# JunweiLiang/Multiverse

Measured on AMD Instinct MI355X. Metric: trajectories/sec (8-obs/12-pred, multi-scale 18x32+9x16 grid, greedy forward), higher is better.
Workload: dtype f16x3 (fp32 operands as two pre-scaled fp16 planes, fp32 accumulate and state; winograd F(3,3) over image rows on pre-transformed operands, 1.67 fp16 MFMAs issued per fp32 product over the gate kernels; error vs fp64 within 2x of the fp32-MFMA path's -- asserted under checkpoint-like dynamic range (; 1 GPU; BASELINE configs[1]: multi-scale 18x32+9x16 (scene 36x64x11), batch 64/GPU, fp32 forward-only, beam 1, obs 8 / pred 12; gate convolution on the fp16 matrix pipe (f16x3 split, fp32-class error); batch_per_gpu=64, global_batch=64, obs_len=8, pred_len=12, parallelism=batch-sharded x1, no data-path collective

## Files before the change

multiverse_amd/csrc/decode_tail.h:

```cpp
#pragma once
#include <hip/hip_runtime.h>
#include <stdint.h>

#include "convlstm_mfma.h"
#include "kernels_misc.h"
#include "plane_layout.h"

namespace mv {

constexpr int kTailMax = 4;

__global__ void pack_h2g_kernel(const float* __restrict__ w, float* __restrict__ wq, int C,
                                int P) {
  const int idx = blockIdx.x * blockDim.x + threadIdx.x;
  if (idx >= C * 32) return;
  const int j = idx & 3, l = (idx >> 2) & 63, kk = idx >> 8;
  const int c = kk * 8 + (l >> 5) * 4 + j, col = l & 31;
  float v = 0.f;
  if (col < 9 * P) {
    const int tap = col / P, p = col - tap * P;
    v = w[((size_t)tap * C + c) * P + p];
  }
  wq[idx] = v;
}

struct H2gQProblem {
  const float* h;
  const float* wq;
  float* q;
  int32_t cells, P;
};
struct H2gQGroup {
  H2gQProblem p[kTailMax];
  int32_t block_end[kTailMax];
  int32_t n;
};

template <int NK>
__device__ __forceinline__ void h2g_q_body(const H2gQProblem& a, int block, int C, float* wl) {
  const int lane = threadIdx.x & 63, wave = threadIdx.x >> 6;
  {
    const f32x4* wg = reinterpret_cast<const f32x4*>(a.wq);
    f32x4* wd = reinterpret_cast<f32x4*>(wl);
    for (int i = threadIdx.x; i < C * 8; i += 256) wd[i] = wg[i];
  }
  __syncthreads();
  const int m_wave = block * 128 + wave * 32;
  if (m_wave >= a.cells) return;
  const int m = m_wave + (lane & 31);
  const float* src = a.h + (size_t)(m < a.cells ? m : 0) * C + (lane >> 5) * 4;
  const f32x4* wsrc = reinterpret_cast<const f32x4*>(wl) + lane;
  f32x16 acc;
#pragma unroll
  for (int i = 0; i < 16; ++i) acc[i] = 0.f;
  for (int c0 = 0; c0 < C; c0 += NK * 8) {
    f32x4 av[NK];
#pragma unroll
    for (int kk = 0; kk < NK; ++kk) av[kk] = *reinterpret_cast<const f32x4*>(src + c0 + kk * 8);
    __builtin_amdgcn_sched_barrier(0);
#pragma unroll
    for (int kk = 0; kk < NK; ++kk) {
      const f32x4 bv = wsrc[((c0 >> 3) + kk) * 64];
#pragma unroll
      for (int j = 0; j < 4; ++j)
        acc = __builtin_amdgcn_mfma_f32_32x32x2f32(av[kk][j], bv[j], acc, 0, 0, 0);
    }
  }
  const int col = lane & 31, QS = 9 * a.P;
  if (col < QS) {
#pragma unroll
    for (int reg = 0; reg < 16; ++reg) {
      const int row = (reg & 3) + 8 * (reg >> 2) + 4 * (lane >> 5);
      const int mm = m_wave + row;
      if (mm < a.cells) a.q[(size_t)mm * QS + col] = acc[reg];
    }
  }
}

template <int NK>
__global__ __launch_bounds__(256)
void h2g_q_kernel(const H2gQGroup g, int C) {
  extern __shared__ __attribute__((aligned(16))) float h2g_wlds[];
  int block = blockIdx.x;
  int pi = 0;
#pragma unroll
  for (int i = 0; i < kTailMax - 1; ++i)
    if (i + 1 < g.n && (int)blockIdx.x >= g.block_end[i]) pi = i + 1;
  if (pi > 0) block -= g.block_end[pi - 1];
  switch (pi) {
    case 0: h2g_q_body<NK>(g.p[0], block, C, h2g_wlds); break;
    case 1: h2g_q_body<NK>(g.p[1], block, C, h2g_wlds); break;
    case 2: h2g_q_body<NK>(g.p[2], block, C, h2g_wlds); break;
    default: h2g_q_body<NK>(g.p[3], block, C, h2g_wlds); break;
  }
}

static inline void launch_h2g_q(const H2gQProblem* probs, int n, int C, hipStream_t stream) {
  H2gQGroup g{};
  g.n = n;
  unsigned total = 0;
  for (int i = 0; i < n; ++i) {
    g.p[i] = probs[i];
    total += (unsigned)((probs[i].cells + 127) / 128);
    g.block_end[i] = (int32_t)total;
  }
  for (int i = n; i < kTailMax; ++i) g.block_end[i] = (int32_t)total;
  const size_t lds = (size_t)C * 128;
  if (C % 256 == 0)
    hipLaunchKernelGGL(h2g_q_kernel<32>, dim3(total), dim3(256), lds, stream, g, C);
  else
    hipLaunchKernelGGL(h2g_q_kernel<16>, dim3(total), dim3(256), lds, stream, g, C);
}

__device__ __forceinline__ void emb_store8(float* __restrict__ x, _Float16* p16, size_t pst,
                                           size_t m, int c8, int E, const float (&v)[8]) {
  f32x4 lo = {v[0], v[1], v[2], v[3]}, hi = {v[4], v[5], v[6], v[7]};
  f32x4* dst = reinterpret_cast<f32x4*>(x + m * E + c8 * 8);
  dst[0] = lo; dst[1] = hi;
  if (p16) {
    typedef _Float16 h8 __attribute__((ext_vector_type(8)));
    h8 a, b;
    const size_t o = plane_index((long long)m, c8 * 8, E);
    if (pst == 0) {
#pragma unroll
      for (int j = 0; j < 8; ++j) a[j] = bf16_half_bits(v[j]);
      *reinterpret_cast<h8*>(p16 + o) = a;
      return;
    }
#pragma unroll
    for (int j = 0; j < 8; ++j) {
      const float s = v[j] * 256.0f;
      const _Float16 h0 = (_Float16)s;
      a[j] = h0;
      b[j] = (_Float16)(s - (float)h0);
    }
    *reinterpret_cast<h8*>(p16 + o) = a;
    *reinterpret_cast<h8*>(p16 + pst + o) = b;
  }
}

__global__ __launch_bounds__(256)
void grid_emb_onehot8_kernel(const int32_t* __restrict__ ids, int ids_stride, int ids_div,
                             const float* __restrict__ w, const float* __restrict__ b,
                             float* __restrict__ out, int M, int H, int W, int E,
                             _Float16* p16, size_t p16_stride, int act = 0) {
  const int ng = E >> 3;
  const size_t item = (size_t)blockIdx.x * blockDim.x + threadIdx.x;
  const int K = H * W;
  if (item >= (size_t)M * K * ng) return;
  const int c8 = (int)(item % ng);
  const size_t mc = item / ng;
  const int m = (int)(mc / K), cell = (int)(mc - (size_t)m * K);
  const int yy = cell / W, xx = cell - yy * W;
  const int id = ids[(size_t)(m / ids_div) * ids_stride];
  const int py = id / W, px = id - py * W;
  const int dy = yy - py, dx = xx - px;
  const bool hot = dy >= -1 && dy <= 1 && dx >= -1 && dx <= 1;
  const float* wp = w + (hot ? (1 - dy) * 3 + (1 - dx) : 4) * E + c8 * 8;
  float v[8];
#pragma unroll
  for (int j = 0; j < 8; ++j) {
    const float acc = hot ? wp[j] : 0.f;
    v[j] = act_apply(act, acc + b[c8 * 8 + j]);
  }
  emb_store8(out, p16, p16_stride, mc, c8, E, v);
}

struct TailProblem {
  const float* q;
  float* out;
  int64_t out_row_stride;
  int32_t* ids_out;
  const float* emb_w;
  const float* emb_b;
  float* x_out;
  _Float16* x16;
  int64_t x16_stride;
  int32_t rows, H, W, P, E;
  int32_t onehot;
  int32_t act;
};
struct TailGroup {
  TailProblem p[kTailMax];
  int32_t block_end[kTailMax];
  int32_t n;
};

__device__ __forceinline__ void decode_tail_body(const TailProblem& a, int row, float* sm) {
  const int tid = threadIdx.x, lane = tid & 63, wave = tid >> 6;
  const int H = a.H, W = a.W, K = H * W, P = a.P, E = a.E, QS = 9 * P;
  float* vals = sm;
  float* wl = sm + 2 * 1024;
  float* red = wl + 9 * 2 * E;
  int* redi = reinterpret_cast<int*>(red + 16);
  const float* qrow = a.q + (size_t)row * K * QS;
  if (a.emb_w && !a.onehot)
    for (int i = tid; i < 9 * P * E; i += blockDim.x) wl[i] = a.emb_w[i];
  float best = -INFINITY;
  int bi = 0x7fffffff;
  for (int idx = tid; idx < K * P; idx += blockDim.x) {
    const int cell = idx / P, p = idx - cell * P;
    const int y = cell / W, x = cell - y * W;
    float acc = 0.f;
#pragma unroll
    for (int t = 0; t < 9; ++t) {
      const int yy = y + t / 3 - 1, xx = x + t % 3 - 1;
      if (yy >= 0 && yy < H && xx >= 0 && xx < W)
        acc += qrow[(size_t)(yy * W + xx) * QS + t * P + p];
    }
    vals[idx] = acc;
    a.out[(size_t)row * a.out_row_stride + idx] = acc;
    if (acc > best || (acc == best && idx < bi)) { best = acc; bi = idx; }
  }
  if (!a.emb_w && !a.ids_out) return;
  int hot = 0;
  if (a.onehot) {
#pragma unroll
    for (int off = 32; off > 0; off >>= 1) {
      const float ov = __shfl_xor(best, off, 64);
      const int oi = __shfl_xor(bi, off, 64);
      if (ov > best || (ov == best && oi < bi)) { best = ov; bi = oi; }
    }
    if (lane == 0) { red[wave] = best; redi[wave] = bi; }
    __syncthreads();
    best = red[0]; bi = redi[0];
    for (int wv = 1; wv < (int)(blockDim.x >> 6); ++wv) {
      const float ov = red[wv];
      const int oi = redi[wv];
      if (ov > best || (ov == best && oi < bi)) { best = ov; bi = oi; }
    }
    hot = bi;
    if (a.ids_out && tid == 0) a.ids_out[row] = hot;
  } else {
    __syncthreads();
  }
  if (!a.emb_w) return;
  const int ng = E >> 3;
  const int py = hot / W, px = hot - py * W;
  for (int item = tid; item < K * ng; item += blockDim.x) {
    const int cell = item / ng, c8 = item - cell * ng;
    const int y = cell / W, x = cell - y * W;
    float v[8];
    if (a.onehot) {
      const int dy = y - py, dx = x - px;
      const bool in = dy >= -1 && dy <= 1 && dx >= -1 && dx <= 1;
      const float* wp = a.emb_w + (in ? (1 - dy) * 3 + (1 - dx) : 4) * E + c8 * 8;
#pragma unroll
      for (int j = 0; j < 8; ++j) v[j] = act_apply(a.act, (in ? wp[j] : 0.f) + a.emb_b[c8 * 8 + j]);
    } else {
      float acc[8];
#pragma unroll
      for (int j = 0; j < 8; ++j) acc[j] = 0.f;
      for (int t = 0; t < 9; ++t) {
        const int yy = y + t / 3 - 1, xx = x + t % 3 - 1;
        if (yy < 0 || yy >= H || xx < 0 || xx >= W) continue;
        const float* ip = vals + (yy * W + xx) * P;
        for (int p = 0; p < P; ++p) {
          const float iv = ip[p];
          const float* wp = wl + (t * P + p) * E + c8 * 8;
#pragma unroll
          for (int j = 0; j < 8; ++j) acc[j] = fmaf(iv, wp[j], acc[j]);
        }
      }
#pragma unroll
      for (int j = 0; j < 8; ++j) v[j] = act_apply(a.act, acc[j] + a.emb_b[c8 * 8 + j]);
    }
    emb_store8(a.x_out, a.x16, (size_t)a.x16_stride, (size_t)row * K + cell, c8, E, v);
  }
}

static inline size_t tail_lds_bytes(int E) {
  return ((size_t)2 * 1024 + (size_t)9 * 2 * E + 32) * sizeof(float);
}
constexpr int kTailThreads = 1024;

__global__ __launch_bounds__(kTailThreads)
void decode_tail_kernel(const TailGroup g) {
  extern __shared__ __attribute__((aligned(16))) float tail_sm[];
  int block = blockIdx.x;
  int pi = 0;
#pragma unroll
  for (int i = 0; i < kTailMax - 1; ++i)
    if (i + 1 < g.n && (int)blockIdx.x >= g.block_end[i]) pi = i + 1;
  if (pi > 0) block -= g.block_end[pi - 1];
  switch (pi) {
    case 0: decode_tail_body(g.p[0], block, tail_sm); break;
    case 1: decode_tail_body(g.p[1], block, tail_sm); break;
    case 2: decode_tail_body(g.p[2], block, tail_sm); break;
    default: decode_tail_body(g.p[3], block, tail_sm); break;
  }
}

static inline void launch_decode_tail(const TailProblem* probs, int n, hipStream_t stream) {
  TailGroup g{};
  g.n = n;
  unsigned total = 0;
  for (int i = 0; i < n; ++i) {
    g.p[i] = probs[i];
    total += (unsigned)probs[i].rows;
    g.block_end[i] = (int32_t)total;
  }
  for (int i = n; i < kTailMax; ++i) g.block_end[i] = (int32_t)total;
  int emax = 32;
  for (int i = 0; i < n; ++i) emax = probs[i].E > emax ? probs[i].E : emax;
  hipLaunchKernelGGL(decode_tail_kernel, dim3(total), dim3(kTailThreads), tail_lds_bytes(emax),
                     stream, g);
}

}
```

multiverse_amd/csrc/engine_forward.h:

```cpp
#pragma once

namespace {


using mv::ConvLstmArgs;

void set_sparse_x(mv_engine* e, ScaleState& S, ConvLstmArgs& a, bool decoder,
                  const int32_t* hot, int hot_stride, int hot_div) {
  a.sx_bias = decoder ? S.sx_dec_bias.p : nullptr;
  a.sx_corr = decoder ? S.sx_dec_corr.p : S.sx_enc_corr.p;
  a.sx_hot = hot; a.sx_hot_stride = hot_stride; a.sx_hot_div = hot_div;
  a.sx_cellyx = S.sx_cellyx.p;
  a.sx_rad = decoder ? 2 : 1;
  a.sx_by_class = decoder ? 1 : 0;
}

ConvLstmArgs conv_problem(mv_engine* e, const ConvCell& cc, const float* x,
                          const float* h, const float* c, const int32_t* src_row_h,
                          const int32_t* src_row_c, float* h_out, float* c_out,
                          int rows, int H, int W, bool zero_state,
                          size_t x_row_stride = 0, bool want_h16 = true) {
  ConvLstmArgs a{};
  const size_t xrs = x_row_stride ? x_row_stride : (size_t)H * W * cc.Cx;
  MV_REQUIRE((size_t)rows * H * W * e->cfg.hidden_size < ((size_t)1 << 31) &&
// ... 243 lines not shown
    launch(e, "wino3_transform", 0, tr3_bytes, [&] {
      mv::launch_wino3_transforms(tr3.data(), (int)tr3.size(), e->issue);
    });
  launch(e, "convlstm_step", g.flops, g.bytes, [&] {
    launch_gate_group(pl, g.p16.data(), packs, w_hwio, v3x, v3h, n, e->issue);
  }, g.dense, pl.mfma_factor);
}

void run_conv_group_f16x3(mv_engine* e, const std::vector<ConvLstmArgs>& probs) {
  const GatePrep g = prepare_gate_group(e, probs);
  const GatePrep* gp = &g;
  issue_gate_group(e, g, plan_gate_groups(e, &gp, 1));
}

void run_conv_group(mv_engine* e, const std::vector<ConvLstmArgs>& probs) {
  if (probs.empty()) return;
  if (e->compute_mode != 0) {
    run_conv_group_f16x3(e, probs);
    return;
  }
  double flops = 0, bytes = 0, dense = 0;
  gate_group_cost(probs, flops, bytes, dense);
  if (e->cfg.convlstm_kernel != 3) {
    const double kk = (double)e->cfg.convlstm_kernel * e->cfg.convlstm_kernel / 9.0;
    launch(e, "convlstm_step", flops * kk, bytes, [&] {
      for (const auto& a : probs) {
        mv::ConvGenericArgs ga{};
        ga.f = a;
        ga.w = cell_of_bias(e, a.bias)->kernel->dev.p;
        ga.ksize = e->cfg.convlstm_kernel;
        mv::launch_convlstm_generic_step(ga, e->issue);
      }
    }, dense * kk, 0.0);
    return;
  }
  launch(e, "convlstm_step", flops, bytes, [&] {
    mv::launch_convlstm_steps(probs.data(), (int)probs.size(), e->issue);
  }, dense, 1.0);
}

void run_conv_pairs(mv_engine* e, const std::vector<ConvLstmArgs>& a,
                    const std::vector<ConvLstmArgs>& b) {
  if (e->compute_mode == 0 || a.empty() || b.empty()) {
    { IssueOn on(e, 0); run_conv_group(e, a); }
    { IssueOn on(e, 1); run_conv_group(e, b); }
    return;
  }
  MV_REQUIRE(a.size() <= 2 && b.size() <= 2, "internal: chain pairs of %zu / %zu problems",
             a.size(), b.size());
  GatePrep ga, gb;
  { IssueOn on(e, 0); ga = prepare_gate_group(e, a); }
  { IssueOn on(e, 1); gb = prepare_gate_group(e, b); }
  const GatePrep* both[2] = {&gb, &ga};
  const ForwardPlan pl = plan_gate_groups(e, both, 2);
  { IssueOn on(e, 0); issue_gate_group(e, ga, pl); }
  { IssueOn on(e, 1); issue_gate_group(e, gb, pl); }
}

void run_scene(mv_engine* e) {
  const mv_config& c = e->cfg;
  const int U = e->num_frames;
  const float* in = e->scene_feat.p;
  int Hi = c.scene_h, Wi = c.scene_w, Ci = c.scene_class;
  const int k = c.scene_conv_kernel;
  for (int i = 0; i < c.num_scales; ++i) {
    const int Ho = e->conv_h[i], Wo = e->conv_w[i], Co = c.scene_conv_dim;
    const int pad_h = std::max((Ho - 1) * 2 + k - Hi, 0);
    const int pad_w = std::max((Wo - 1) * 2 + k - Wi, 0);
    const size_t total = (size_t)U * Ho * Wo * Co;
    float* out = e->scene_conv[i].p;
    const float *w = e->scene_W[i]->dev.p, *b = e->scene_b[i]->dev.p;
    if (k == 1 && Co <= 64) {
      const size_t M = (size_t)U * Ho * Wo;
      launch(e, "scene_proj1x1_mfma", 2.0 * M * Ci * Co,
             4.0 * (total + (double)M * Ci), [&] {
        hipLaunchKernelGGL(mv::scene_proj1x1_mfma_kernel, dim3(cdiv(M, 128)), dim3(256), 0,
                           e->issue, in, w, b, out, U, Hi, Wi, Ci, Ho, Wo, Co, c.activation);
      });
    } else {
    launch(e, "scene_conv_s2_tanh", 2.0 * total * k * k * Ci,
           4.0 * (total + (double)U * Hi * Wi * Ci), [&] {
      hipLaunchKernelGGL(mv::scene_conv_s2_tanh_kernel, dim3(cdiv(total, 256)),
                         dim3(256), 0, e->issue, in, w, b, out, U, Hi, Wi, Ci,
                         Ho, Wo, Co, k, pad_h / 2, pad_w / 2, c.activation);
    });
    }
    in = out; Hi = Ho; Wi = Wo; Ci = Co;
  }
  for (int s = 0; s < c.num_scales; ++s) {
    ScaleState& S = e->sc[s];
    if (!S.use) continue;
    const size_t total = (size_t)c.batch_size * S.K * c.scene_conv_dim;
    launch(e, "scene_mean", (double)total * c.obs_len,
           4.0 * total * (c.obs_len + 1), [&] {
      hipLaunchKernelGGL(mv::scene_mean_kernel, dim3(cdiv(total, 256)), dim3(256),
                         0, e->issue, e->scene_conv[s].p, e->obs_scene.p,
                         S.scene_mean.p, c.batch_size, c.obs_len, S.K,
                         c.scene_conv_dim);
    });
  }
}

struct Cursors {
  int cls[MV_MAX_SCALES] = {0, 0};
  int reg[MV_MAX_SCALES] = {0, 0};
};

static bool beam_shared_first() {
  static const bool on =
      !(getenv("MV_BEAM_SHARED_FIRST") && atoi(getenv("MV_BEAM_SHARED_FIRST")) == 0);
  return on;
}

enum : int { kChainCls = 1, kChainReg = 2, kChainAll = 3 };

void encoder_step_problems(mv_engine* e, Cursors& cur, int t, int chains,
                           std::vector<ConvLstmArgs>& probs) {
  const mv_config& c = e->cfg;
  const int N = c.batch_size, T = c.obs_len, D = c.scene_conv_dim;
  for (int s = 0; s < c.num_scales; ++s) {
    {
      ScaleState& S = e->sc[s];
      if (!S.use) continue;
      if (chains & kChainCls) {
      const size_t total = (size_t)N * S.K * D;
      const bool sparse = sparse_x_on(e, S);
      const size_t nc = (size_t)N * 9 * 4 * c.hidden_size;
      if (e->no_scene()) {
        if (!sparse) {
          const int E = S.enc_cls.Cx;
          const size_t tx = (size_t)N * S.K * E;
          launch(e, "enc_grid_emb_onehot", (double)tx, 4.0 * tx, [&] {
            size_t pst = 0;
            _Float16* p16 = e->plane_out(S.xbuf_cls.p, &pst);
            hipLaunchKernelGGL(mv::enc_grid_emb_onehot_kernel, dim3(cdiv(tx, 256)), dim3(256),
                               0, e->issue, S.labels.p, T, t, 1, e->enc_emb_W->dev.p,
                               e->enc_emb_b->dev.p, S.xbuf_cls.p, N, S.H, S.W, E, p16, pst,
                               c.activation);
          });
        }
      } else if (sparse) {
        if (t == 0)
          launch(e, "sx_encoder_corr", 2.0 * nc * D * T, 4.0 * nc * T, [&] {
            hipLaunchKernelGGL(mv::sx_encoder_corr_kernel,
                               dim3(cdiv((size_t)4 * c.hidden_size, 256), 9,
                                    cdiv((size_t)N, mv::kSxRows) * T),
                               dim3(256), 0, e->issue, S.enc_cls.kernel->dev.p,
                               e->scene_conv[s].p, e->obs_scene.p, S.labels.p, N, T, -1, S.K, D,
                               c.hidden_size, S.sx_enc_corr.p);
          });
      } else {
      launch(e, "enc_class_input", 0, 4.0 * total, [&] {
        size_t pst = 0;
        _Float16* p16 = e->plane_out(S.xbuf_cls.p, &pst);
        hipLaunchKernelGGL(mv::enc_class_input_kernel, dim3(cdiv(total, 256)),
                           dim3(256), 0, e->issue, e->scene_conv[s].p,
                           e->obs_scene.p, S.labels.p, S.xbuf_cls.p, N, T, t, S.K, D, p16,
                           pst);
      });
      }
      const int cc = cur.cls[s];
      probs.push_back(conv_problem(e, S.enc_cls, S.xbuf_cls.p, S.cls_h[cc].p,
                                   S.cls_c[cc].p, nullptr, nullptr, S.cls_h[cc ^ 1].p,
                                   S.cls_c[cc ^ 1].p, N, S.H, S.W, t == 0, 0,
                                   t + 1 < T || !c.use_gnn));
      probs.back().skip_h32 =
          (t + 1 < T || (!c.use_gnn && (c.beam_size == 1 || beam_shared_first()))) ? 1 : 0;
      if (sparse && e->no_scene()) {
        set_sparse_x(e, S, probs.back(), true, S.labels.p + t, T, 1);
        probs.back().sx_bias = S.sx_enc_bias.p;
        probs.back().sx_corr = S.sx_enc_tab.p;
      } else if (sparse) {
        set_sparse_x(e, S, probs.back(), false, S.labels.p + t, T, 1);
        probs.back().sx_corr = S.sx_enc_corr.p + (size_t)t * nc;
      }
      cur.cls[s] ^= 1;
      }
      if (!(chains & kChainReg)) continue;
      const size_t row = (size_t)S.K * 2;
      const int cr = cur.reg[s];
      if (!c.use_single_decoder)
        probs.push_back(conv_problem(e, S.enc_reg, S.obs_reg.p + (size_t)t * row,
                                     S.reg_h[cr].p, S.reg_c[cr].p, nullptr, nullptr,
                                     S.reg_h[cr ^ 1].p, S.reg_c[cr ^ 1].p, N, S.H, S.W,
                                     t == 0, (size_t)T * row));
      if (!c.use_single_decoder) probs.back().skip_h32 = 1;
      cur.reg[s] ^= 1;
    }
  }
}

void run_encoders(mv_engine* e, Cursors& cur, bool pairs) {
  for (int t = 0; t < e->cfg.obs_len; ++t) {
    if (!pairs) {
      std::vector<ConvLstmArgs> probs;
      encoder_step_problems(e, cur, t, kChainAll, probs);
      run_conv_group(e, probs);
      continue;
    }
    std::vector<ConvLstmArgs> pa, pb;
    { IssueOn on(e, 0); encoder_step_problems(e, cur, t, kChainCls, pa); }
    { IssueOn on(e, 1); encoder_step_problems(e, cur, t, kChainReg, pb); }
    run_conv_pairs(e, pa, pb);
  }
}

static int gnn_version() {
  const char* v = getenv("MV_GNN");
  if (v && strcmp(v, "v1") == 0) return 1;
  if (v && strcmp(v, "v2") == 0) return 2;
  return 3;
}

struct GnnJob {
  ScaleState* S; const float* h; const int32_t* src_row; float* out; int rows, sm_div;
  const int32_t* row_ref = nullptr;
};

void run_gnn_jobs(mv_engine* e, const std::vector<GnnJob>& jobs) {
  const mv_config& c = e->cfg;
  static const int env_ver = gnn_version();
  const size_t max_rows = (size_t)c.batch_size * (size_t)std::max(1, c.beam_size);
  auto v3_ok = [&](const GnnJob& J) {
    return (gnn_scene_dim(e) == 0 || gnn_scene_dim(e) == 64) &&
           max_rows * J.S->K * c.hidden_size * 4 < ((size_t)1 << 32);
  };
  for (size_t j0 = 0; j0 < jobs.size();) {
    const GnnJob& A = jobs[j0];
    const bool tiled = env_ver >= 2 && A.S->W <= 32 && c.hidden_size == 256 && c.scene_conv_dim <= 64;
    size_t nj = 1;
    if (tiled && j0 + 1 < jobs.size() && jobs[j0 + 1].S->W <= 32) nj = 2;
    const int ver = env_ver >= 3 && !(v3_ok(A) && (nj == 1 || v3_ok(jobs[j0 + 1]))) ? 2 : env_ver;
    mv::GnnGroup grp{};
    double flops = 0, bytes = 0;
    unsigned nblocks = 0;
    for (size_t j = 0; j < nj; ++j) {
      const GnnJob& J = jobs[j0 + j];
      const size_t cells = (size_t)J.rows * J.S->K;
      size_t pst = 0;
      _Float16* p16 = e->plane_out(J.out, &pst);
      const bool need_f32 = !(tiled && p16 && !e->train && e->compute_mode != 0);
      flops += cells * (9.0 * 2 * 2 * (c.hidden_size + gnn_scene_dim(e)) +
                        9.0 * 2 * c.hidden_size);
      bytes += 4.0 * cells * c.hidden_size *
                   (1.0 + (need_f32 ? 1.0 : 0.0) + (p16 ? 1.0 : 0.0)) +
               4.0 * (cells / J.sm_div) * gnn_scene_dim(e);
      int ng = 0;
      const unsigned nb = ver >= 3 ? mv::gnn_v3_blocks(cells, &ng) : mv::gnn_v2_blocks(cells, &ng);
      mv::GnnProblem& P = grp.p[j];
      P.h = J.h; P.scene_mean = J.S->scene_mean.p; P.src_row = J.src_row;
      P.out = need_f32 ? J.out : nullptr; P.p16 = p16; P.p16_stride = pst;
      P.M = J.rows; P.H = J.S->H; P.W = J.S->W; P.sm_div = J.sm_div; P.ngroups = ng;
      P.row_ref = J.row_ref;
      if (j == 0) grp.nblocks0 = nb;
      nblocks += nb;
    }
    if (nj == 1) grp.nblocks0 = nblocks;
    launch(e, "gnn_attend", flops, bytes, [&] {
      if (tiled && ver >= 3) {
        hipLaunchKernelGGL(mv::gnn_attend_v3_kernel, dim3(nblocks), dim3(mv::kGnn3Threads), 0,
                           e->issue, grp, c.hidden_size, gnn_scene_dim(e));
      } else if (tiled) {
        hipLaunchKernelGGL(mv::gnn_attend_v2_kernel, dim3(nblocks), dim3(mv::kGnnThreads), 0, e->issue,
                           grp, c.hidden_size, gnn_scene_dim(e));
      } else {
        const size_t cells = (size_t)A.rows * A.S->K;
        size_t pst = 0;
        _Float16* p16 = e->plane_out(A.out, &pst);
        if (c.hidden_size <= 256)
          hipLaunchKernelGGL(mv::gnn_attend_kernel<1>, dim3(cdiv(cells, 4)), dim3(256), 0,
                             e->issue, A.h, A.S->scene_mean.p, A.src_row, A.out, A.rows,
                             A.S->H, A.S->W, c.hidden_size, gnn_scene_dim(e), A.sm_div, p16, pst);
        else
          hipLaunchKernelGGL(mv::gnn_attend_kernel<2>, dim3(cdiv(cells, 4)), dim3(256), 0,
                             e->issue, A.h, A.S->scene_mean.p, A.src_row, A.out, A.rows,
                             A.S->H, A.S->W, c.hidden_size, gnn_scene_dim(e), A.sm_div, p16, pst);
      }
    });
    j0 += nj;
  }
}

void run_gnn(mv_engine* e, ScaleState& S, const float* h, const int32_t* src_row,
             float* out, int rows, int sm_div) {
  run_gnn_jobs(e, {GnnJob{&S, h, src_row, out, rows, sm_div}});
}

template <int P>
void run_hidden2grid(mv_engine* e, ScaleState& S, const float* h, const float* w,
                     float* out, size_t out_row_stride, int rows) {
  const size_t cells = (size_t)rows * S.K;
  const int C = e->cfg.hidden_size;
  launch(e, "hidden2grid", cells * 2.0 * 9 * C * P, 4.0 * cells * (C + P), [&] {
    hipLaunchKernelGGL(mv::hidden2grid_kernel<P>, dim3(cdiv(cells, 4)), dim3(256),
                       0, e->issue, h, w, out, out_row_stride, rows, S.H, S.W, C);
  });
}

static bool tail_v2() {
  static const bool on = !(getenv("MV_TAIL") && strcmp(getenv("MV_TAIL"), "v1") == 0);
  return on;
}

void run_emb_onehot(mv_engine* e, ScaleState& S, const int32_t* ids, int stride,
                    float* out, int rows, int ids_div = 1) {
  const int E = e->cfg.emb_size;
  const size_t total = (size_t)rows * S.K * E;
  launch(e, "grid_emb_onehot", (double)total, 4.0 * total, [&] {
    size_t pst = 0;
    _Float16* p16 = e->plane_out(out, &pst);
    if (tail_v2() && E % 8 == 0)
      hipLaunchKernelGGL(mv::grid_emb_onehot8_kernel, dim3(cdiv(total / 8, 256)), dim3(256), 0,
                         e->issue, ids, stride, ids_div, S.emb_cls_W->dev.p,
                         S.emb_cls_b->dev.p, out, rows, S.H, S.W, E, p16, pst, e->cfg.activation);
    else
      hipLaunchKernelGGL(mv::grid_emb_onehot_kernel, dim3(cdiv(total, 256)),
                         dim3(256), 0, e->issue, ids, stride, ids_div, S.emb_cls_W->dev.p,
                         S.emb_cls_b->dev.p, out, rows, S.H, S.W, E, p16, pst, e->cfg.activation);
  });
}

void run_emb_dense(mv_engine* e, ScaleState& S, const float* x, size_t row_stride,
                   float* out, int rows, Param* W = nullptr, Param* b = nullptr, int P = 2) {
  const int E = e->cfg.emb_size;
  const size_t total = (size_t)rows * S.K * E;
  if (!W) { W = S.emb_reg_W; b = S.emb_reg_b; }
  launch(e, "grid_emb_dense", total * 2.0 * 9 * P, 4.0 * total, [&] {
    size_t pst = 0;
    _Float16* p16 = e->plane_out(out, &pst);
    hipLaunchKernelGGL(mv::grid_emb_dense_kernel, dim3(cdiv(total, 256)), dim3(256),
                       0, e->issue, x, row_stride, W->dev.p, b->dev.p, out, rows, S.H, S.W,
                       P, E, p16, pst, e->cfg.activation);
  });
}

ConvLstmArgs reg_decoder_problem(mv_engine* e, int s, Cursors& cur, int t, int Tp,
                                 bool embed = true) {
  const mv_config& c = e->cfg;
  ScaleState& S = e->sc[s];
  const int N = c.batch_size, T = c.obs_len;
  const size_t orow = (size_t)Tp * S.K * 2;
  if (t == 0)
    run_emb_dense(e, S, S.obs_reg.p + (size_t)(T - 1) * S.K * 2, (size_t)T * S.K * 2,
                  S.xbuf_reg.p, N);
  else if (embed)
    run_emb_dense(e, S, S.out_reg.p + (size_t)(t - 1) * S.K * 2, orow, S.xbuf_reg.p, N);
  const int cr = cur.reg[s];
  cur.reg[s] ^= 1;
  return conv_problem(e, S.dec_reg, S.xbuf_reg.p, S.reg_h[cr].p, S.reg_c[cr].p, nullptr,
                      nullptr, S.reg_h[cr ^ 1].p, S.reg_c[cr ^ 1].p, N, S.H, S.W, false);
}

void reg_decoder_output(mv_engine* e, int s, const Cursors& cur, int t, int Tp) {
  ScaleState& S = e->sc[s];
  const size_t orow = (size_t)Tp * S.K * 2;
  run_hidden2grid<2>(e, S, S.reg_h[cur.reg[s]].p, S.out_reg_W->dev.p,
                     S.out_reg.p + (size_t)t * S.K * 2, orow, e->cfg.batch_size);
}

struct TailPlan {
  int s;
  const float* cls_h; int cls_rows; float* cls_out; int64_t cls_stride;
  bool cls_next;
  const float* reg_h; float* reg_out; int64_t reg_stride; bool reg_next;
  int reg_rows = 0;
  int32_t* cls_ids_out = nullptr; float* cls_x_out = nullptr; float* reg_x_out = nullptr;
  bool cls_embed = true;
  bool do_cls = true, do_reg = true;
};

void run_tail(mv_engine* e, const std::vector<TailPlan>& plans) {
  const mv_config& c = e->cfg;
  const int C = c.hidden_size, E = c.emb_size, N = c.batch_size;
  std::vector<mv::H2gQProblem> qp;
  std::vector<mv::TailProblem> tp;
  double qbytes = 0, qflops = 0, tbytes = 0;
  for (const TailPlan& pl : plans) {
    ScaleState& S = e->sc[pl.s];
    MV_REQUIRE((size_t)S.K * 2 <= 2048 && E % 16 == 0 && E <= 512,
               "decode tail: K %d / emb_size %d", S.K, E);
    const int reg_rows = pl.reg_rows ? pl.reg_rows : N;
    const size_t cc = (size_t)pl.cls_rows * S.K, cr = (size_t)reg_rows * S.K;
    if (pl.do_cls) {
      qp.push_back(mv::H2gQProblem{pl.cls_h, S.wq_cls.p, S.q_cls.p, (int32_t)cc, 1});
      qbytes += 4.0 * cc * (C + 9.0);
      qflops += 2.0 * 9 * C * cc;
    }
    if (pl.do_reg) {
      qp.push_back(mv::H2gQProblem{pl.reg_h, S.wq_reg.p, S.q_reg.p, (int32_t)cr, 2});
      qbytes += 4.0 * cr * (C + 18.0);
      qflops += 2.0 * 9 * C * 2.0 * cr;
    }
    if (pl.do_cls) {
    mv::TailProblem a{};
    a.q = S.q_cls.p; a.out = pl.cls_out; a.out_row_stride = pl.cls_stride;
    a.rows = pl.cls_rows; a.H = S.H; a.W = S.W; a.P = 1; a.E = E; a.onehot = 1;
    a.act = c.activation;
    tbytes += 4.0 * cc * (9 + 1);
    if (pl.cls_next) {
      a.ids_out = pl.cls_ids_out ? pl.cls_ids_out : S.ids.p;
      if (pl.cls_x_out) {
        if (pl.cls_embed) {
          a.emb_w = S.emb_cls_W->dev.p; a.emb_b = S.emb_cls_b->dev.p;
          a.x_out = pl.cls_x_out;
          tbytes += 4.0 * cc * E;
        }
      } else if (!sparse_x_on(e, S)) {
        size_t pst = 0;
        a.emb_w = S.emb_cls_W->dev.p; a.emb_b = S.emb_cls_b->dev.p;
        a.x_out = S.xbuf_cls.p;
        a.x16 = e->plane_out(S.xbuf_cls.p, &pst); a.x16_stride = (int64_t)pst;
        tbytes += 4.0 * cc * E * (a.x16 ? 2 : 1);
      }
    }
    tp.push_back(a);
    }
    if (!pl.do_reg) continue;
    mv::TailProblem b{};
    b.q = S.q_reg.p; b.out = pl.reg_out; b.out_row_stride = pl.reg_stride;
    b.rows = reg_rows; b.H = S.H; b.W = S.W; b.P = 2; b.E = E; b.onehot = 0;
    b.act = c.activation;
    tbytes += 4.0 * cr * (18 + 2);
    if (pl.reg_next) {
      size_t pst = 0;
      b.emb_w = S.emb_reg_W->dev.p; b.emb_b = S.emb_reg_b->dev.p;
      if (pl.reg_x_out) {
        b.x_out = pl.reg_x_out;
        tbytes += 4.0 * cr * E;
      } else {
      b.x_out = S.xbuf_reg.p;
      b.x16 = e->plane_out(S.xbuf_reg.p, &pst); b.x16_stride = (int64_t)pst;
      tbytes += 4.0 * cr * E * (b.x16 ? 2 : 1);
      }
    }
    tp.push_back(b);
  }
  MV_REQUIRE(qp.size() <= (size_t)mv::kTailMax, "decode tail: too many chains");
  if (qp.empty()) return;
  launch(e, "hidden2grid", qflops, qbytes, [&] {
    mv::launch_h2g_q(qp.data(), (int)qp.size(), C, e->issue);
  });
  launch(e, "decode_tail", 0, tbytes, [&] {
    mv::launch_decode_tail(tp.data(), (int)tp.size(), e->issue);
  });
}

void run_decoders_greedy(mv_engine* e, Cursors& cur, int Tp, bool pairs) {
  const mv_config& c = e->cfg;
  const int N = c.batch_size, T = c.obs_len;
  const bool v2 = tail_v2();
  MV_REQUIRE(!pairs || (v2 && !c.use_single_decoder), "internal: chain pairs need the grouped "
             "decoder tail and a regression decoder");
  for (int t = 0; t < Tp; ++t) {
    auto step_problems = [&](int chains, std::vector<ConvLstmArgs>& probs) {
      if ((chains & kChainCls) && c.use_gnn) {
        std::vector<GnnJob> jobs;
        for (int s = 0; s < c.num_scales; ++s)
          if (e->sc[s].use)
            jobs.push_back(GnnJob{&e->sc[s], e->sc[s].cls_h[cur.cls[s]].p, nullptr,
                                  e->sc[s].cls_hg.p, N, 1});
        run_gnn_jobs(e, jobs);
      }
      for (int s = 0; s < c.num_scales; ++s) {
        ScaleState& S = e->sc[s];
        if (!S.use) continue;
        if (chains & kChainCls) {
          const int cc = cur.cls[s];
          const float* hin = c.use_gnn ? S.cls_hg.p : S.cls_h[cc].p;
          const bool sparse = sparse_x_on(e, S) && (t == 0 || !c.class_feedback_dense);
          if (sparse)
            ;
          else if (t == 0)
            run_emb_onehot(e, S, S.labels.p + (T - 1), T, S.xbuf_cls.p, N);
          else if (c.class_feedback_dense)
            run_emb_dense(e, S, S.out_cls.p + (size_t)(t - 1) * S.K, (size_t)Tp * S.K,
                          S.xbuf_cls.p, N, S.emb_cls_W, S.emb_cls_b, 1);
          else if (!v2)
            run_emb_onehot(e, S, S.ids.p, 1, S.xbuf_cls.p, N);
          probs.push_back(conv_problem(e, S.dec_cls, S.xbuf_cls.p, hin, S.cls_c[cc].p,
                                       nullptr, nullptr, S.cls_h[cc ^ 1].p,
                                       S.cls_c[cc ^ 1].p, N, S.H, S.W, false, 0,
                                       !c.use_gnn));
          if (sparse) {
            if (t == 0) set_sparse_x(e, S, probs.back(), true, S.labels.p + (T - 1), T, 1);
            else set_sparse_x(e, S, probs.back(), true, S.ids.p, 1, 1);
          }
          cur.cls[s] ^= 1;
        }
        if ((chains & kChainReg) && !c.use_single_decoder)
          probs.push_back(reg_decoder_problem(e, s, cur, t, Tp, !v2));
      }
      std::stable_sort(probs.begin(), probs.end(), [](const ConvLstmArgs& a, const ConvLstmArgs& b) {
        return (a.sx_corr == nullptr) > (b.sx_corr == nullptr);
      });
    };
    auto step_tail = [&](int chains) {
      std::vector<TailPlan> plans;
      for (int s = 0; s < c.num_scales; ++s) {
        ScaleState& S = e->sc[s];
        if (!S.use) continue;
        TailPlan pl{};
        pl.s = s;
        pl.cls_h = S.cls_h[cur.cls[s]].p; pl.cls_rows = N;
        pl.cls_out = S.out_cls.p + (size_t)t * S.K; pl.cls_stride = (int64_t)Tp * S.K;
        pl.cls_next = t + 1 < Tp && !c.class_feedback_dense;
        pl.reg_h = S.reg_h[cur.reg[s]].p;
        pl.reg_out = S.out_reg.p + (size_t)t * S.K * 2; pl.reg_stride = (int64_t)Tp * S.K * 2;
        pl.reg_next = t + 1 < Tp;
        if (c.use_single_decoder) {
          pl.reg_h = pl.cls_h;
          pl.reg_next = false;
        }
        pl.do_cls = (chains & kChainCls) != 0;
        pl.do_reg = (chains & kChainReg) != 0;
        plans.push_back(pl);
      }
      run_tail(e, plans);
    };
    if (pairs) {
      std::vector<ConvLstmArgs> pa, pb;
      { IssueOn on(e, 0); step_problems(kChainCls, pa); }
      { IssueOn on(e, 1); step_problems(kChainReg, pb); }
      run_conv_pairs(e, pa, pb);
      { IssueOn on(e, 0); step_tail(kChainCls); }
      { IssueOn on(e, 1); step_tail(kChainReg); }
      continue;
    }
    std::vector<ConvLstmArgs> probs;
    step_problems(kChainAll, probs);
    run_conv_group(e, probs);
    if (v2) {
      step_tail(kChainAll);
      continue;
    }
    for (int s = 0; s < c.num_scales; ++s) {
      ScaleState& S = e->sc[s];
      if (!S.use) continue;
      const size_t orow = (size_t)Tp * S.K;
      float* logits = S.out_cls.p + (size_t)t * S.K;
      run_hidden2grid<1>(e, S, S.cls_h[cur.cls[s]].p, S.out_cls_W->dev.p, logits, orow, N);
      if (t + 1 < Tp && !c.class_feedback_dense) {
        launch(e, "argmax_rows", 0, 4.0 * N * S.K, [&] {
          hipLaunchKernelGGL(mv::argmax_rows_kernel, dim3(N), dim3(64), 0, e->issue,
                             logits, orow, S.ids.p, N, S.K);
        });
      }
      if (c.use_single_decoder)
        run_hidden2grid<2>(e, S, S.cls_h[cur.cls[s]].p, S.out_reg_W->dev.p,
                           S.out_reg.p + (size_t)t * S.K * 2, (size_t)Tp * S.K * 2, N);
      else
        reg_decoder_output(e, s, cur, t, Tp);
    }
  }
}

__global__ void tile_rows_kernel(const float* __restrict__ in, float* __restrict__ out,
                                 size_t row_elems4, int B, size_t total4) {
  const size_t idx = (size_t)blockIdx.x * blockDim.x + threadIdx.x;
  if (idx >= total4) return;
  const size_t r = idx / row_elems4, off = idx - r * row_elems4;
  reinterpret_cast<mv::f32x4_t*>(out)[idx] =
      reinterpret_cast<const mv::f32x4_t*>(in)[(r / B) * row_elems4 + off];
}

__global__ void tile_beam0_kernel(float* __restrict__ logits, int K, int B, size_t total) {
  const size_t idx = (size_t)blockIdx.x * blockDim.x + threadIdx.x;
  if (idx >= total) return;
  const size_t r = idx / K;
  if (r % B) logits[idx] = logits[(r - r % B) * K + (idx - r * K)];
}

__global__ void beam_backtrace_kernel(const int32_t* __restrict__ step_ids,
                                      const int32_t* __restrict__ step_parents,
                                      int32_t* __restrict__ out_ids,
                                      int32_t* __restrict__ trace, int N, int B,
                                      int T) {
  const int idx = blockIdx.x * blockDim.x + threadIdx.x;
  if (idx >= N * B) return;
  const int n = idx / B, b = idx - n * B;
  int par = b;
  for (int t = T - 1; t >= 0; --t) {
    const size_t o = ((size_t)t * N + n) * B + par;
    out_ids[((size_t)n * B + b) * T + t] = step_ids[o];
    trace[((size_t)n * B + b) * T + t] = par;
    par = step_parents[o];
  }
}

__global__ void beam_gather_logits_kernel(const float* __restrict__ step_logits,
                                          const int32_t* __restrict__ trace,
                                          float* __restrict__ out, int N, int B,
                                          int T, int K) {
  const size_t idx = (size_t)blockIdx.x * blockDim.x + threadIdx.x;
  const size_t total = (size_t)N * B * T * K;
  if (idx >= total) return;
  const int k = idx % K;
  size_t r = idx / K;
  const int t = r % T; r /= T;
  const int b = r % B;
  const int n = r / B;
  const int par = trace[((size_t)n * B + b) * T + t];
  out[idx] = step_logits[(((size_t)t * N + n) * B + par) * K + k];
}

void run_decoders_beam(mv_engine* e, int s, Cursors& cur, int Tp) {
  const mv_config& c = e->cfg;
  ScaleState& S = e->sc[s];
  const int N = c.batch_size, T = c.obs_len, B = c.beam_size, K = S.K,
            C = c.hidden_size;
  const int R = N * B;
  const bool shared_first = beam_shared_first();
  if (!shared_first) {
    const int cc = cur.cls[s];
    const size_t row4 = (size_t)K * C / 4, total4 = (size_t)R * row4;
    launch(e, "beam_tile_state", 0, 8.0 * total4 * 16, [&] {
      hipLaunchKernelGGL(tile_rows_kernel, dim3(cdiv(total4, 256)), dim3(256), 0,
                         e->issue, S.cls_h[cc].p, S.cls_h[cc ^ 1].p, row4, B, total4);
      hipLaunchKernelGGL(tile_rows_kernel, dim3(cdiv(total4, 256)), dim3(256), 0,
                         e->issue, S.cls_c[cc].p, S.cls_c[cc ^ 1].p, row4, B, total4);
    });
    e->plane_invalidate(S.cls_h[cc ^ 1].p);
    cur.cls[s] ^= 1;
  }
  HIP_CHECK(hipMemsetAsync(e->bm_lp[0].p, 0, (size_t)R * sizeof(float), e->issue));
  int lpi = 0;
  const int32_t* src = nullptr;
  const bool sparse = sparse_x_on(e, S);
  static const bool dedupe_env =
      !(getenv("MV_BEAM_GNN_DEDUPE") && atoi(getenv("MV_BEAM_GNN_DEDUPE")) == 0);
  const bool dedupe = dedupe_env && shared_first && c.use_gnn && K <= 64 * mv::kBeamRankJ &&
                      !(getenv("MV_BEAM_STEP") && strcmp(getenv("MV_BEAM_STEP"), "v1") == 0) &&
                      !(getenv("MV_GNN") && strcmp(getenv("MV_GNN"), "v1") == 0);
  for (int time = 0; time <= Tp; ++time) {
    const bool one_per_sample = shared_first && time <= 1;
    const int rows_now = one_per_sample ? N : R;
    if (time > 0) {
      const int cc = cur.cls[s];
      const float* hin = c.use_gnn ? S.cls_hg.p : S.cls_h[cc].p;
      std::vector<ConvLstmArgs> probs;
      probs.push_back(conv_problem(e, S.dec_cls, S.xbuf_cls.p, hin, S.cls_c[cc].p,
                                   (c.use_gnn && !dedupe) ? nullptr : src, src,
                                   S.cls_h[cc ^ 1].p, S.cls_c[cc ^ 1].p, rows_now, S.H, S.W,
                                   false, 0, !c.use_gnn));
      if (sparse) {
        if (time == 1)
          set_sparse_x(e, S, probs.back(), true, S.labels.p + (T - 1), T, one_per_sample ? 1 : B);
        else
          set_sparse_x(e, S, probs.back(), true, e->bm_ids.p + (size_t)(time - 2) * R, 1, 1);
      }
      cur.cls[s] ^= 1;
      const bool v2 = tail_v2();
      const bool single = c.use_single_decoder != 0;
      MV_REQUIRE(!single || v2, "use_single_decoder with beam search needs the v2 decoder tail");
      if (!single) probs.push_back(reg_decoder_problem(e, s, cur, time - 1, Tp, !v2));
      run_conv_group(e, probs);
      float* logits = e->bm_logits.p + (size_t)(time - 1) * R * K;
      float* regstep = single ? e->bm_reg_steps.p + (size_t)(time - 1) * R * K * 2 : nullptr;
      const size_t lrow = one_per_sample ? (size_t)B * K : (size_t)K;
      if (v2) {
        TailPlan pl{};
        pl.s = s;
        pl.cls_h = S.cls_h[cur.cls[s]].p; pl.cls_rows = rows_now;
        pl.cls_out = logits; pl.cls_stride = lrow; pl.cls_next = false;
        if (single) {
          pl.reg_h = pl.cls_h; pl.reg_rows = rows_now;
          pl.reg_out = regstep; pl.reg_stride = (int64_t)lrow * 2; pl.reg_next = false;
        } else {
        pl.reg_h = S.reg_h[cur.reg[s]].p;
        pl.reg_out = S.out_reg.p + (size_t)(time - 1) * K * 2;
        pl.reg_stride = (int64_t)Tp * K * 2; pl.reg_next = time < Tp;
        }
        run_tail(e, {pl});
      } else {
        reg_decoder_output(e, s, cur, time - 1, Tp);
        run_hidden2grid<1>(e, S, S.cls_h[cur.cls[s]].p, S.out_cls_W->dev.p, logits,
                           lrow, rows_now);
      }
      if (one_per_sample) {
        const size_t total = (size_t)R * K;
        hipLaunchKernelGGL(tile_beam0_kernel, dim3(cdiv(total, 256)), dim3(256), 0,
                           e->issue, logits, K, B, total);
        if (single)
          hipLaunchKernelGGL(tile_beam0_kernel, dim3(cdiv(total * 2, 256)), dim3(256), 0,
                             e->issue, regstep, K * 2, B, total * 2);
      }
      int32_t* ids = e->bm_ids.p + (size_t)(time - 1) * R;
      int32_t* parents = e->bm_parents.p + (size_t)(time - 1) * R;
      if (dedupe)
        HIP_CHECK(hipMemsetAsync(e->bm_ref.p, 0, (size_t)R * sizeof(int32_t), e->issue));
      launch(e, "beam_step", 0, 4.0 * R * K, [&] {
        launch_beam_step(e->issue, logits, e->bm_lp[lpi].p, e->bm_cand.p, N, B, K, time,
                         c.diverse_beam, logf(c.diverse_gamma), c.fix_num_timestep,
                         e->bm_lp[lpi ^ 1].p, ids, parents, e->bm_src_row.p,
                         one_per_sample ? 1 : B, dedupe ? e->bm_ref.p : nullptr);
      });
      lpi ^= 1;
      src = e->bm_src_row.p;
      if (time == Tp) break;
      if (!sparse) run_emb_onehot(e, S, ids, 1, S.xbuf_cls.p, R);
    } else if (sparse) {
    } else if (shared_first) {
      run_emb_onehot(e, S, S.labels.p + (T - 1), T, S.xbuf_cls.p, N, 1);
    } else {
      run_emb_onehot(e, S, S.labels.p + (T - 1), T, S.xbuf_cls.p, R, B);
    }
    if (c.use_gnn) {
      if (dedupe) {
        GnnJob job{&S, S.cls_h[cur.cls[s]].p, nullptr, S.cls_hg.p, rows_now,
                   one_per_sample ? 1 : B};
        job.row_ref = time >= 2 ? e->bm_ref.p : nullptr;
        run_gnn_jobs(e, {job});
      } else {
      const int out_rows = (shared_first && time == 0) ? N : R;
      run_gnn(e, S, S.cls_h[cur.cls[s]].p, src, S.cls_hg.p, out_rows,
              (shared_first && time == 0) ? 1 : B);
      }
    }
  }
  hipLaunchKernelGGL(beam_backtrace_kernel, dim3(cdiv(R, 256)), dim3(256), 0,
                     e->issue, e->bm_ids.p, e->bm_parents.p, e->bm_out_ids.p,
                     e->bm_trace.p, N, B, Tp);
  const size_t total = (size_t)R * Tp * K;
  hipLaunchKernelGGL(beam_gather_logits_kernel, dim3(cdiv(total, 256)), dim3(256), 0,
                     e->issue, e->bm_logits.p, e->bm_trace.p, e->bm_out_logits.p,
                     N, B, Tp, K);
  if (c.use_single_decoder) {
    const size_t tot2 = (size_t)R * Tp * K * 2;
    hipLaunchKernelGGL(beam_gather_logits_kernel, dim3(cdiv(tot2, 256)), dim3(256), 0,
                       e->issue, e->bm_reg_steps.p, e->bm_trace.p, e->bm_out_reg.p,
                       N, B, Tp, K * 2);
  }
  if (lpi != 0)
    HIP_CHECK(hipMemcpyAsync(e->bm_lp[0].p, e->bm_lp[1].p, (size_t)R * sizeof(float),
                             hipMemcpyDeviceToDevice, e->issue));
}

constexpr int kChainPairMaxBatch = 64;

void enqueue_forward(mv_engine* e, bool beam, bool capturing = false) {
  const mv_config& c = e->cfg;
  const int Tp = e->pred_len;
  const bool pairs = !beam && e->stream_b && !e->profiling && !capturing && c.beam_size == 1 &&
                     !c.use_single_decoder && tail_v2() && c.batch_size <= kChainPairMaxBatch;
  Cursors cur;
  if (pairs) {
    ChainFork fork(e);
    if (!e->no_scene()) { IssueOn on(e, 0); run_scene(e); }
    run_encoders(e, cur, true);
    run_decoders_greedy(e, cur, Tp, true);
    HIP_CHECK(hipGetLastError());
    return;
  }
  if (!e->no_scene()) run_scene(e);
  run_encoders(e, cur, false);
  if (beam) {
    int s = 0;
    for (int i = 0; i < c.num_scales; ++i) if (e->sc[i].use) s = i;
    run_decoders_beam(e, s, cur, Tp);
  } else {
    run_decoders_greedy(e, cur, Tp, false);
  }
  HIP_CHECK(hipGetLastError());
}

void run_forward(mv_engine* e, bool beam) {
  MV_REQUIRE(e->inputs_ready, "no inputs uploaded (mv_upload_inputs)");
  ensure_params(e);
  if (beam)
    MV_REQUIRE(e->cfg.beam_size > 1, "engine was created with beam_size 1");
  if (!e->graph_mode || e->profiling) {
    enqueue_forward(e, beam);
    e->last_forward = beam ? 2 : 1;
    return;
  }
  const auto key = std::make_tuple(beam ? 1 : 0, e->pred_len, e->num_frames);
  auto it = e->graphs.find(key);
  if (it == e->graphs.end()) {
    hipGraph_t g = nullptr;
    HIP_CHECK(hipStreamBeginCapture(e->stream, hipStreamCaptureModeThreadLocal));
    try {
      enqueue_forward(e, beam, true);
    } catch (...) {
      (void)hipStreamEndCapture(e->stream, &g);
      if (g) (void)hipGraphDestroy(g);
      throw;
    }
    HIP_CHECK(hipStreamEndCapture(e->stream, &g));
    hipGraphExec_t ex = nullptr;
    hipError_t ie = hipGraphInstantiate(&ex, g, nullptr, nullptr, 0);
    (void)hipGraphDestroy(g);
    HIP_CHECK(ie);
    it = e->graphs.emplace(key, ex).first;
  }
  HIP_CHECK(hipGraphLaunch(it->second, e->stream));
  e->last_forward = beam ? 2 : 1;
}

}
```

Before: 4326 trajectories/sec.

## Fuse hidden2grid MFMA projection into decode tail kernel via LDS

Adds a fused tail kernel in which each block computes its row's hidden-to-grid projection with fp32 MFMA into LDS and then runs the existing decode tail body on that LDS buffer. This removes a separate kernel launch and the global write and readback of the q intermediate for greedy decoding. It applies by default for non-pair greedy steps when total rows are at most 1024, C is a multiple of 128 and the LDS budget fits. The cost is that each block recomputes the projection with only one block per CU under a large LDS allocation, which may lower occupancy compared with the separate grid-wide GEMM. A nounroll pragma is also added to the embedding inner loop.

Result: no change. 4332 trajectories/sec (median of 6 runs) (+0.1%).

```diff
diff --git a/multiverse_amd/csrc/decode_tail.h b/multiverse_amd/csrc/decode_tail.h
--- a/multiverse_amd/csrc/decode_tail.h
+++ b/multiverse_amd/csrc/decode_tail.h
@@ -186,14 +186,14 @@
   int32_t n;
 };
 
-__device__ __forceinline__ void decode_tail_body(const TailProblem& a, int row, float* sm) {
+__device__ __forceinline__ void decode_tail_body(const TailProblem& a, int row, float* sm,
+                                                 const float* qrow) {
   const int tid = threadIdx.x, lane = tid & 63, wave = tid >> 6;
   const int H = a.H, W = a.W, K = H * W, P = a.P, E = a.E, QS = 9 * P;
   float* vals = sm;
   float* wl = sm + 2 * 1024;
   float* red = wl + 9 * 2 * E;
   int* redi = reinterpret_cast<int*>(red + 16);
-  const float* qrow = a.q + (size_t)row * K * QS;
   if (a.emb_w && !a.onehot)
     for (int i = tid; i < 9 * P * E; i += blockDim.x) wl[i] = a.emb_w[i];
   float best = -INFINITY;
@@ -255,6 +255,7 @@
         const int yy = y + t / 3 - 1, xx = x + t % 3 - 1;
         if (yy < 0 || yy >= H || xx < 0 || xx >= W) continue;
         const float* ip = vals + (yy * W + xx) * P;
+#pragma nounroll
         for (int p = 0; p < P; ++p) {
           const float iv = ip[p];
           const float* wp = wl + (t * P + p) * E + c8 * 8;
@@ -273,6 +274,10 @@
   return ((size_t)2 * 1024 + (size_t)9 * 2 * E + 32) * sizeof(float);
 }
 constexpr int kTailThreads = 1024;
+
+__device__ __forceinline__ const float* tail_q_row(const TailProblem& a, int row) {
+  return a.q + (size_t)row * a.H * a.W * 9 * a.P;
+}
 
 __global__ __launch_bounds__(kTailThreads)
 void decode_tail_kernel(const TailGroup g) {
@@ -284,10 +289,10 @@
     if (i + 1 < g.n && (int)blockIdx.x >= g.block_end[i]) pi = i + 1;
   if (pi > 0) block -= g.block_end[pi - 1];
   switch (pi) {
-    case 0: decode_tail_body(g.p[0], block, tail_sm); break;
-    case 1: decode_tail_body(g.p[1], block, tail_sm); break;
-    case 2: decode_tail_body(g.p[2], block, tail_sm); break;
-    default: decode_tail_body(g.p[3], block, tail_sm); break;
+    case 0: decode_tail_body(g.p[0], block, tail_sm, tail_q_row(g.p[0], block)); break;
+    case 1: decode_tail_body(g.p[1], block, tail_sm, tail_q_row(g.p[1], block)); break;
+    case 2: decode_tail_body(g.p[2], block, tail_sm, tail_q_row(g.p[2], block)); break;
+    default: decode_tail_body(g.p[3], block, tail_sm, tail_q_row(g.p[3], block)); break;
   }
 }
 
@@ -307,4 +312,122 @@
                      stream, g);
 }
 
-}
+struct FusedTailProblem {
+  TailProblem t;
+  const float* h;
+  const float* wq;
+};
+struct FusedTailGroup {
+  FusedTailProblem p[kTailMax];
+  int32_t block_end[kTailMax];
+  int32_t n;
+  int32_t q_off, w_off;
+};
+
+constexpr int kFusedNK = 16;
+
+__device__ __forceinline__ void fused_tail_body(const FusedTailProblem& f, int row, int C,
+                                                float* sm, int q_off, int w_off) {
+  const TailProblem& a = f.t;
+  const int lane = threadIdx.x & 63, wave = threadIdx.x >> 6;
+  const int K = a.H * a.W, QS = 9 * a.P;
+  float* ql = sm + q_off;
+  float* wl = sm + w_off;
+  {
+    const f32x4* wg = reinterpret_cast<const f32x4*>(f.wq);
+    f32x4* wd = reinterpret_cast<f32x4*>(wl);
+    for (int i = threadIdx.x; i < C * 8; i += kTailThreads) wd[i] = wg[i];
+  }
+  __syncthreads();
+  const float* himg = f.h + (size_t)row * K * C;
+  const f32x4* wsrc = reinterpret_cast<const f32x4*>(wl) + lane;
+  const int col = lane & 31;
+  for (int m_wave = wave * 32; m_wave < K; m_wave += (kTailThreads / 64) * 32) {
+    const int m = m_wave + (lane & 31);
+    const float* src = himg + (size_t)(m < K ? m : 0) * C + (lane >> 5) * 4;
+    f32x16 acc;
+#pragma unroll
+    for (int i = 0; i < 16; ++i) acc[i] = 0.f;
+    for (int c0 = 0; c0 < C; c0 += kFusedNK * 8) {
+      f32x4 av[kFusedNK];
+#pragma unroll
+      for (int kk = 0; kk < kFusedNK; ++kk)
+        av[kk] = *reinterpret_cast<const f32x4*>(src + c0 + kk * 8);
+      __builtin_amdgcn_sched_barrier(0);
+#pragma unroll
+      for (int kk = 0; kk < kFusedNK; ++kk) {
+        const f32x4 bv = wsrc[((c0 >> 3) + kk) * 64];
+#pragma unroll
+        for (int j = 0; j < 4; ++j)
+          acc = __builtin_amdgcn_mfma_f32_32x32x2f32(av[kk][j], bv[j], acc, 0, 0, 0);
+      }
+    }
+    if (col < QS) {
+#pragma unroll
+      for (int reg = 0; reg < 16; ++reg) {
+        const int mm = m_wave + (reg & 3) + 8 * (reg >> 2) + 4 * (lane >> 5);
+        if (mm < K) ql[mm * QS + col] = acc[reg];
+      }
+    }
+  }
+  __syncthreads();
+  decode_tail_body(a, row, sm, ql);
+}
+
+__global__ __launch_bounds__(kTailThreads)
+void fused_tail_kernel(const FusedTailGroup g, int C) {
+  extern __shared__ __attribute__((aligned(16))) float fused_tail_sm[];
+  int block = blockIdx.x;
+  int pi = 0;
+#pragma unroll
+  for (int i = 0; i < kTailMax - 1; ++i)
+    if (i + 1 < g.n && (int)blockIdx.x >= g.block_end[i]) pi = i + 1;
+  if (pi > 0) block -= g.block_end[pi - 1];
+  switch (pi) {
+    case 0: fused_tail_body(g.p[0], block, C, fused_tail_sm, g.q_off, g.w_off); break;
+    case 1: fused_tail_body(g.p[1], block, C, fused_tail_sm, g.q_off, g.w_off); break;
+    case 2: fused_tail_body(g.p[2], block, C, fused_tail_sm, g.q_off, g.w_off); break;
+    default: fused_tail_body(g.p[3], block, C, fused_tail_sm, g.q_off, g.w_off); break;
+  }
+}
+
+constexpr size_t kFusedTailLdsMax = (size_t)160 * 1024;
+
+static inline size_t fused_tail_lds_bytes(const FusedTailProblem* probs, int n, int C,
+                                          int* q_off = nullptr, int* w_off = nullptr) {
+  int emax = 32;
+  size_t qmax = 0;
+  for (int i = 0; i < n; ++i) {
+    const TailProblem& t = probs[i].t;
+    emax = t.E > emax ? t.E : emax;
+    const size_t q = ((size_t)t.H * t.W * 9 * t.P + 3) / 4 * 4;
+    qmax = q > qmax ? q : qmax;
+  }
+  const size_t qo = tail_lds_bytes(emax) / sizeof(float), wo = qo + qmax;
+  if (q_off) *q_off = (int)qo;
+  if (w_off) *w_off = (int)wo;
+  return (wo + (size_t)C * 32) * sizeof(float);
+}
+
+static inline void launch_fused_tail(const FusedTailProblem* probs, int n, int C,
+                                     hipStream_t stream) {
+  static const bool attr = [] {
+    (void)hipFuncSetAttribute(reinterpret_cast<const void*>(fused_tail_kernel),
+                              hipFuncAttributeMaxDynamicSharedMemorySize, (int)kFusedTailLdsMax);
+    return true;
+  }();
+  (void)attr;
+  FusedTailGroup g{};
+  g.n = n;
+  unsigned total = 0;
+  for (int i = 0; i < n; ++i) {
+    g.p[i] = probs[i];
+    total += (unsigned)probs[i].t.rows;
+    g.block_end[i] = (int32_t)total;
+  }
+  for (int i = n; i < kTailMax; ++i) g.block_end[i] = (int32_t)total;
+  const size_t lds = fused_tail_lds_bytes(probs, n, C, &g.q_off, &g.w_off);
+  hipLaunchKernelGGL(fused_tail_kernel, dim3(total), dim3(kTailThreads), lds, stream, g, C);
+}
+
+}
diff --git a/multiverse_amd/csrc/engine_forward.h b/multiverse_amd/csrc/engine_forward.h
--- a/multiverse_amd/csrc/engine_forward.h
+++ b/multiverse_amd/csrc/engine_forward.h
@@ -569,6 +569,17 @@
   return on;
 }
 
+static int tail_fused_mode() {
+  static const int mode = [] {
+    const char* v = getenv("MV_TAIL");
+    if (v && (strcmp(v, "v1") == 0 || strcmp(v, "v2") == 0)) return -1;
+    return (v && strcmp(v, "fused") == 0) ? 1 : 0;
+  }();
+  return mode;
+}
+constexpr int kFusedTailMaxRows = 1024;
+enum TailCaller { kTailOther = 0, kTailGreedy = 1, kTailGreedyPair = 2 };
+
 void run_emb_onehot(mv_engine* e, ScaleState& S, const int32_t* ids, int stride,
                     float* out, int rows, int ids_div = 1) {
   const int E = e->cfg.emb_size;
@@ -636,7 +647,7 @@
   bool do_cls = true, do_reg = true;
 };
 
-void run_tail(mv_engine* e, const std::vector<TailPlan>& plans) {
+void run_tail(mv_engine* e, const std::vector<TailPlan>& plans, TailCaller who = kTailOther) {
   const mv_config& c = e->cfg;
   const int C = c.hidden_size, E = c.emb_size, N = c.batch_size;
   std::vector<mv::H2gQProblem> qp;
@@ -704,6 +715,22 @@
   }
   MV_REQUIRE(qp.size() <= (size_t)mv::kTailMax, "decode tail: too many chains");
   if (qp.empty()) return;
+  if (who != kTailOther && tail_fused_mode() >= 0) {
+    std::vector<mv::FusedTailProblem> fp;
+    long long rows = 0;
+    for (size_t i = 0; i < tp.size(); ++i) {
+      fp.push_back(mv::FusedTailProblem{tp[i], qp[i].h, qp[i].wq});
+      rows += tp[i].rows;
+    }
+    const bool fits = C % 128 == 0 &&
+        mv::fused_tail_lds_bytes(fp.data(), (int)fp.size(), C) <= mv::kFusedTailLdsMax;
+    if (fits && (tail_fused_mode() > 0 || (who == kTailGreedy && rows <= kFusedTailMaxRows))) {
+      launch(e, "decode_tail", qflops, qbytes + tbytes, [&] {
+        mv::launch_fused_tail(fp.data(), (int)fp.size(), C, e->issue);
+      });
+      return;
+    }
+  }
   launch(e, "hidden2grid", qflops, qbytes, [&] {
     mv::launch_h2g_q(qp.data(), (int)qp.size(), C, e->issue);
   });
@@ -782,7 +809,7 @@
         pl.do_reg = (chains & kChainReg) != 0;
         plans.push_back(pl);
       }
-      run_tail(e, plans);
+      run_tail(e, plans, pairs ? kTailGreedyPair : kTailGreedy);
     };
     if (pairs) {
       std::vector<ConvLstmArgs> pa, pb;
```
